# entn-at/exemplars_vc

Hardware: AMD Instinct MI355X
Metric: spectral frames/sec converted (100 NMF iters, N=4096 dict) (higher is better)
Workload: dtype f64

## Files before the change

exemplars_vc_amd/_lib.py:

```python
from __future__ import annotations

import ctypes as C
import os

_HERE = os.path.dirname(os.path.abspath(__file__))
LIB_PATH = os.environ.get("EVC_LIB") or os.path.join(_HERE, "libevc_hip.so")

F64, F32 = 0, 1
FRAME_MAJOR, BIN_MAJOR = 0, 1
EPS_ADD, EPS_ZERO_REPLACE, EPS_NONE, EPS_CLAMP = 0, 1, 2, 3
ALGO_GRAM, ALGO_FACTORED, ALGO_LITERAL, ALGO_AUTO = 0, 1, 2, 3
INIT_GIVEN, INIT_SKLEARN, INIT_CONST = 0, 1, 2
STOP_NONE, STOP_SKLEARN, STOP_PYMF, STOP_DECOMP = 0, 1, 2, 3
PROX_POSITIVE, PROX_SIGNED = 0, 1
PROX_ISTA, PROX_FISTA, PROX_NESTEROV = 0, 1, 2
PROX_LIP_MEAN, PROX_LIP_MAX = 0, 1
LOSS_FROBENIUS, LOSS_KL = 0, 1
FLAG_NO_FUSED, FLAG_EXACT_DIV, FLAG_NO_EXCHANGE, FLAG_NO_ALL_RESIDENT, FLAG_PAIR_TILES, FLAG_NO_LONE_BIN = 1, 2, 4, 16, 32, 64
LEARN_SKLEARN, LEARN_PYMF = 0, 1
CDL_BOTH, CDL_DICT_ONLY = 0, 1
DCL_BOTH, DCL_DICT_ONLY = 0, 1

SYMBOLS = ("evc_version", "evc_strerror", "evc_device_count", "evc_workspace_bytes",
           "evc_nmf_solve", "evc_nmf_convert", "evc_synthesize", "evc_residual",
           "evc_griffin_lim_workspace_bytes", "evc_griffin_lim", "evc_griffin_lim_batch_workspace_bytes",
           "evc_griffin_lim_batch", "evc_dtw_workspace_bytes", "evc_dtw_align",
           "evc_stft_frames", "evc_stft_workspace_bytes", "evc_stft", "evc_dict_bytes", "evc_dict_prepare",
           "evc_dtw_path_rows", "evc_dtw_gather_rows", "evc_cd_workspace_bytes", "evc_cd_solve",
           "evc_learn_workspace_bytes", "evc_learn_splits", "evc_nmf_learn",
           "evc_cd_learn_workspace_bytes", "evc_cd_learn_splits", "evc_cd_learn",
           "evc_mfcc_workspace_bytes", "evc_mfcc", "evc_beta_workspace_bytes", "evc_beta_solve",
           "evc_beta_learn_workspace_bytes", "evc_beta_learn_splits", "evc_beta_learn_route", "evc_beta_learn",
           "evc_online_workspace_bytes", "evc_online_splits", "evc_online_learn",
           "evc_online_transform_workspace_bytes", "evc_online_transform",
           "evc_online_fresh_workspace_bytes", "evc_online_learn_fresh",
           "evc_deconv_workspace_bytes", "evc_deconv_solve", "evc_deconv_synthesize",
           "evc_deconv_learn_workspace_bytes", "evc_deconv_learn_splits", "evc_deconv_learn",
           "evc_semi_workspace_bytes", "evc_semi_solve",
           "evc_prox_workspace_bytes", "evc_prox_solve",
           "evc_prox_masked_workspace_bytes", "evc_prox_masked_solve",
           "evc_prox_learn_workspace_bytes", "evc_prox_learn_block", "evc_prox_learn",
# ... 478 lines not shown
```

exemplars_vc_amd/csrc/evc_api.hip:

```cpp
#include "evc_solve_plan.h"

#include <math.h>
#include <stdlib.h>
#include <string.h>

using namespace evc;

namespace {

constexpr int DICT_MAGIC = 0x45564344;

struct SolveCall {
    const void* A; int lda;
    const void* X; int ldx;
    void* H; int ldh;
    int M, N, T_;
    const int* utt_offsets; int n_utt;
    void* ws; size_t ws_bytes;
    int* n_iter_out; double* err_out;
    const SynthArgs* y;
    hipStream_t s;
};

int copy_back(const UttState& u, int n_utt, int n_slots, int* n_iter_out, double* err_out, hipStream_t s) {
// ... 173 lines not shown
    inf->kernel = r.kernel;
    inf->members = r.members;
    inf->exchange = r.members > 1 ? 1 : 0;
    AbortHook hook(r.members > 1 ? fb.coop_cnt + COOP_MAX_TILES : nullptr, o.test_abort_at);
    HIP_TRY(hook.begin(true, s));
    int first = 1;
    if (o.check_every > 0 && o.stop_rule == EVC_STOP_SKLEARN) {
        HIP_TRY(fused_iterate(w.fl, fb, r, w.u, d.N, d.T_, 0, 1, 1, w.err2, o.eps_mode, o.eps, o.l1, 1, o.loss, s,
                              nullptr));
        HIP_TRY(utt_check(w.err2, w.u, n_utt, 0, o.check_every, o.stop_rule, o.tol, s));
        first = 0;
    }
    if (o.ev_loop_start) HIP_TRY(hipEventRecord((hipEvent_t)o.ev_loop_start, s));
    int done = 0;
    while (done < o.iters) {
        int n = o.iters - done;
        bool check = false;
        if (o.check_every > 0 && n >= o.check_every) { n = o.check_every; check = true; }
        const bool last = r.direct_export && done + n == o.iters;
        HIP_TRY(hook.before_launch(s));
        ++inf->launches;
        HIP_TRY(fused_iterate(w.fl, fb, r, w.u, d.N, d.T_, n, first, check ? 1 : 0, w.err2, o.eps_mode, o.eps, o.l1,
                              o.stop_rule == EVC_STOP_NONE ? 1 : 0, o.loss, s, last ? &lt : nullptr,
                              !(o.reserved & EVC_FLAG_NO_LONE_BIN)));
        first = 0;
        done += n;
        if (check)
            HIP_TRY(utt_check(w.err2, w.u, n_utt, done / o.check_every, o.check_every, o.stop_rule,
                              o.tol, s));
    }
    if (o.ev_loop_stop) HIP_TRY(hipEventRecord((hipEvent_t)o.ev_loop_stop, s));
    return ST_OK;
}

int finish_fused(const Workspace<double>& w, const Dims& d, const evc_solve_opts& o, const FusedTail& t, double* H, int ldh,
                 const SynthArgs* y, int y_members, hipStream_t s) {
    const bool fm = (o.layout == EVC_FRAME_MAJOR);
    if (t.export_h) HIP_TRY(fused_export_h(w.fl, w.fb.Hp, H, ldh, fm ? 1 : 0, d.T_, d.N, s));
    switch (t.y_from) {
        case Y_SLABS:
            return fused_unpack_y(w.flB, w.Yslab, y_members, (long)w.flB.vp, d.T_, y->Mb, static_cast<double*>(y->Y), y->ldy,
                                  fm ? 1 : 0, s);
        case Y_PREPASS:
            return fused_synthesize(w.flB, w.B2p, w.fb.Hp, w.Yp, w.u, d.N, d.T_, y->Mb, static_cast<double*>(y->Y), y->ldy,
                                    fm ? 1 : 0, s);
        case Y_ROWS:
            HIP_TRY(fused_export_h(w.fl, w.fb.Hp, w.H0, d.Np, 1, d.T_, d.N, s));
// ... 515 lines not shown
```

exemplars_vc_amd/csrc/evc_fused.hip:

```cpp
#include "evc_fused_common.h"

namespace evc {

__global__ void k_pack_dict(const double* __restrict__ At, int ldA, int n_rows, int NT, int msteps, int mtiles,
                            double* __restrict__ A1p, double* __restrict__ A2p, int ones_bin) {
    const long gid = (long)blockIdx.x * blockDim.x + threadIdx.x;
    const int msp = (msteps + 1) & ~1;
    const long n1 = (long)NT * msp * 64, n2 = (long)NT * mtiles * 4 * 64;
    if (gid < n1) {
        const int e = gid & 1, l = (gid >> 1) & 63, s = 2 * (int)((gid >> 7) % (msp / 2)) + e;
        const long j = (gid >> 7) / (msp / 2);
        const int i = l & 15;
        const long n = 16 * j + 4 * (i & 3) + (i >> 2);
        const int bin = bin_of(s, l >> 4);
        if (A1p) A1p[gid] = (s < msteps && bin == ones_bin) ? 1.0 : ((s < msteps && n < n_rows) ? At[n * ldA + bin] : 0.0);
    } else if (gid < n1 + n2) {
        const long g = gid - n1;
        const int e = g & 1, l = (g >> 1) & 63, r = 2 * (int)((g >> 7) & 1) + e, u = (g >> 8) % mtiles;
        const long j = (g >> 8) / mtiles;
        const long n = 16 * j + 4 * (l >> 4) + r;
        if (A2p) A2p[g] = n < n_rows ? At[n * ldA + 16 * u + (l & 15)] : 0.0;
    }
}

// ... 409 lines not shown

static hipError_t launch_general(const FusedLayout& f, const FusedArgs& a, int c_req, hipStream_t s) {
    const int C = a.skip_all_live ? 1 : (c_req > 0 ? c_req : (f.TT >= 1024 ? 2 : 1));
    switch (C) {
        case 1: return dispatch_msteps<1>(f.msteps, a, s);
        case 2: return dispatch_msteps<2>(f.msteps, a, s);
        default: return hipErrorInvalidValue;
    }
}

static FusedArgs fused_args(const FusedLayout& f, const double* A1p, const double* A2p, const double* Xp, const double* Hp,
                            double* Vp, const UttState& u, int N, int T_, int iters, int first) {
    FusedArgs a{};
    a.A1p = A1p; a.A2p = A2p; a.Xp = Xp; a.Hp = reinterpret_cast<f64x2*>(const_cast<double*>(Hp)); a.Vp = Vp;
    a.frame_utt = u.frame_utt; a.active = u.active;
    a.NT = f.NT; a.TT = f.TT; a.N = N; a.T_ = T_; a.M = f.M;
    a.iters = iters; a.first = first;
    a.coop_c = 1; a.spare_q = -1;
    return a;
}

hipError_t fused_iterate(const FusedLayout& f, const FusedBuffers& b, const FusedRoute& r, const UttState& u, int N,
                         int T_, int iters, int first, int write_err, double* err2, int eps_mode, double eps, double l1,
                         int all_live_known, int loss, hipStream_t s, const FusedLaunchTail* tail, bool lone_bin) {
    FusedArgs a = fused_args(f, b.A1p, b.A2p, b.Xp, b.Hp, b.Vp, u, N, T_, iters, first);
    a.err2 = err2; a.write_err = write_err;
    a.loss = loss; a.exact_div = r.exact_div;
    a.eps_mode = eps_mode; a.eps = eps; a.l1 = l1;
    const bool xy = r.kernel == EVC_KERNEL_FUSED_XY;
    const bool all_res = xy || r.kernel == EVC_KERNEL_FUSED_ALL;
    if (r.kernel == EVC_KERNEL_FUSED_MU) return launch_general(f, a, r.c_req, s);
    if (first && all_res && r.init_const && iters > 0) {
        a.init_const = 1; a.h0 = u.h0; a.rsum = b.rsum;
    } else if (first) {
        FusedArgs p = a;
        p.iters = 0;
        p.write_err = (iters == 0) ? write_err : 0;
        hipError_t e = launch_general(f, p, 1, s);
        if (e != hipSuccess) return e;
        a.first = 0;
    }
    if (iters == 0) return hipSuccess;
    hipError_t e;
    if (all_res) {
        a.coop_c = r.members; a.coop_buf = b.coop_buf; a.coop_cnt = b.coop_cnt;
        a.coop_abort = b.coop_cnt + COOP_MAX_TILES;
        if (all_live_known && tail) {
            a.Hx = tail->Hx; a.ldhx = tail->ldhx; a.hx_frame_major = tail->hx_frame_major;
            a.hx_wide = (a.Hx && a.hx_frame_major && !(reinterpret_cast<uintptr_t>(a.Hx) & 15) && !(a.ldhx & 1)) ? 1 : 0;
            if (!xy) {
                a.Yb2p = tail->Yb2p; a.Yslab = tail->Yslab; a.y_stride = tail->y_stride; a.y_mt = tail->y_mt;
                a.skip_hp = tail->skip_hp;
            }
        }
        e = xy ? fused_xy_launch(f.msteps, a, r.n_cus, s) : fused_all_launch(f.msteps, a, r.n_cus, s, lone_bin);
        a.coop_c = 1;
        a.first = 0; a.init_const = 0; a.Hx = nullptr; a.Yslab = nullptr; a.skip_hp = 0;
    } else {
        if (r.members > 1) {
            a.coop_c = r.members; a.coop_buf = b.coop_buf; a.coop_cnt = b.coop_cnt;
            a.coop_abort = b.coop_cnt + COOP_MAX_TILES;
        }
        e = fused_res_launch(f.msteps, a, s);
    }
    if (e != hipSuccess || all_live_known) return e;
    a.skip_all_live = 1;
    return launch_general(f, a, 1, s);
}

hipError_t fused_synthesize(const FusedLayout& fB, const double* B2p, const double* Hp, double* Yp,
                            const UttState& u, int N, int T_, int Mb, double* Y, long ldy, int frame_major,
                            hipStream_t s) {
    FusedArgs a = fused_args(fB, B2p, B2p, Yp, Hp, Yp, u, N, T_, 0, 1);
    a.force_live = 1; a.loss = EVC_LOSS_FROBENIUS; a.eps_mode = EVC_EPS_ADD;
    hipError_t e = dispatch_msteps<1>(fB.msteps, a, s);
    if (e != hipSuccess) return e;
    return fused_unpack_y(fB, Yp, 1, 0, T_, Mb, Y, ldy, frame_major, s);
}
// ... 11 lines not shown
```

exemplars_vc_amd/csrc/evc_fused_all_body.inc:

```
#if EVC_ALL_LONE
template <int MSTEPS, int C>
__global__ __launch_bounds__(ATHREADS, 2) void k_fused_lone(FusedArgs a) {
    constexpr bool KL = false, LONE = true;
    static_assert(MSTEPS > 4 && C > 1 && AllShape<MSTEPS, C, false>::LDS_DICT, "two bin tiles, the dictionary in LDS, direct exchange");
#else
template <int MSTEPS, int C, bool KL>
__global__ __launch_bounds__(ATHREADS, 2) void k_fused_all(FusedArgs a) {
    constexpr bool LONE = false;
#endif
    using S = AllShape<MSTEPS, C, KL>;
    constexpr int DS = LONE ? MSTEPS - 1 : MSTEPS;
    constexpr int MT = S::MT;
    constexpr int E = S::E;
    constexpr int NE = S::NE;
    constexpr int RSTR = S::RSTR;
    constexpr int MSP = (MSTEPS + 1) & ~1;
    constexpr int PR = S::PR;
    constexpr int TPD = 16 * PR;
    __shared__ __attribute__((aligned(16))) double s_red[2][AW * RSTR];
    __shared__ __attribute__((aligned(16))) double s_v[2][E];
    __shared__ __attribute__((aligned(16))) double s_x[2][E];
    __shared__ __attribute__((aligned(16))) double s_r[2][KL ? E : 1];
    __shared__ double s_stage[2][S::STG];
    __shared__ double s_dict[S::LDS_DICT ? ATILES * TPD : 1];
    __shared__ unsigned s_hb[2];
    __shared__ int s_fail;
    const int tid = threadIdx.x, lane = tid & 63;
    const int w8 = __builtin_amdgcn_readfirstlane(tid >> 6);
    const int half = w8 >> 2, w = w8 & 3, th = tid & (AW * 64 - 1);
    const int CR = C > 0 ? C : a.coop_c;
    const int member = blockIdx.x % CR;
    const int g = 2 * (blockIdx.x / CR) + half;
    double* const red = s_red[half];
    double* const vL = s_v[half];
    double* const xL = s_x[half];
    double* const rL = s_r[half];
    double* const stage = s_stage[half];
    unsigned hb = 0;
    const double* __restrict__ A1p = a.A1p;
    const double* __restrict__ A2p = a.A2p;
    f64x2* __restrict__ Hp = a.Hp;
    const int NT = a.NT;
    const long tile0 = (long)member * ATILES + w;
    const unsigned ul = (unsigned)lane;
    long sw = 0;

    const __amdgpu_buffer_rsrc_t r1 = __builtin_amdgcn_make_buffer_rsrc(const_cast<double*>(A1p), 0, NT * (MSP * 512), 0x00020000);
    const __amdgpu_buffer_rsrc_t r2 = __builtin_amdgcn_make_buffer_rsrc(const_cast<double*>(A2p), 0, NT * (MT * 2048), 0x00020000);
    const __amdgpu_buffer_rsrc_t rx = __builtin_amdgcn_make_buffer_rsrc(a.coop_buf, 0, C > 1 ? 2 * a.groups * (C * 4096) : 0, 0x00020000);
// ... 54 lines not shown
                }
            return;
        }
#ifdef EVC_ALL_NOFRAG
        if (nofrag_go) return;
#endif
        const int so = (int)(tile0 + sw + AW * k) * (MT * 2048);
#pragma unroll
        for (int u = 0; u < MT; ++u)
#pragma unroll
            for (int r = 0; r < 4; r += 2) {
                const f64x2 v = __builtin_bit_cast(f64x2, __builtin_amdgcn_raw_buffer_load_b128(r2, ul16 + (u * 2 + (r >> 1)) * 1024, so, 0));
                a2[u][r] = v[0];
                a2[u][r + 1] = v[1];
            }
    };

    const int mode = a.eps_mode;
    const double eps = a.eps;
    const double d0 = a.l1 + (mode == EVC_EPS_ADD ? a.eps : 0.0);
    const f64x4 dinit = {d0, d0, d0, d0};
    const unsigned lo = fast_lo(mode, eps);
    unsigned seq = 0;
    int rs_es = 1, rs_len = 0, rs_pub0 = 0, rs_pub1 = 0, rs_src0 = -1, rs_src1 = -1, rs_src2 = -1;
    if (C < 0) {
        rs_es = (NE + CR - 1) / CR;
        rs_len = NE - member * rs_es;
        rs_len = rs_len < 0 ? 0 : (rs_len > rs_es ? rs_es : rs_len);
        const int e0 = th, e1 = th + AW * 64;
        const int j0 = e0 / rs_es, j1 = (e1 < NE ? e1 : e0) / rs_es;
        rs_pub0 = (j0 * CR + member) * rs_es + (e0 - j0 * rs_es);
        rs_pub1 = (j1 * CR + member) * rs_es + ((e1 < NE ? e1 : e0) - j1 * rs_es);
        auto src = [&](int idx) {
            if (idx >= CR * rs_es) return -1;
            const int el = idx % rs_es;
            return el < rs_len ? member * CR * rs_es + idx : -1;
        };
        rs_src0 = src(th);
        rs_src1 = src(th + AW * 64);
        rs_src2 = src(th + 2 * AW * 64);
    }
    if (tid == 0) s_fail = 0;
    if (tid < 2) s_hb[tid] = 0;

    if (a.stagger_cycles > 0 && ((blockIdx.x / CR) & 1)) {
        const long long t0 = __builtin_amdgcn_s_memtime();
// ... 31 lines not shown
            }
            const double hv = h0_of(lane & 15);
#pragma unroll
            for (int k = 0; k < AKT; ++k) {
                const long n0 = 16 * (tile0 + AW * k) + 4 * (lane >> 4);
#pragma unroll
                for (int r = 0; r < 4; ++r) h[k][r] = n0 + r < a.N ? hv : 0.0;
            }
        } else if (valid) {
            for (int e = th; e < E; e += AW * 64) {
                const int s = e >> 6, l = e & 63;
                const bool in = s < MSTEPS;
                xL[e] = in ? a.Xp[(tt * MSTEPS + s) * 64 + l] : 0.0;
                vL[e] = in ? a.Vp[(tt * 8 + s) * 64 + l] : 0.0;
                if (KL) rL[e] = xL[e] / (vL[e] < a.eps ? a.eps : vL[e]);
            }
#pragma unroll
            for (int k = 0; k < AKT; ++k) {
                const f64x2* t = Hp + (tt * NT + tile0 + AW * k) * 128;
                const f64x2 h01 = t[ul], h23 = t[ul + 64];
                h[k][0] = h01[0]; h[k][1] = h01[1]; h[k][2] = h23[0]; h[k][3] = h23[1];
            }
        }
        __syncthreads();
        if (valid && !KL) {
            double x[DS], xl = 0.0;
#pragma unroll
            for (int s = 0; s < DS; ++s) x[s] = xL[s * 64 + lane];
            if constexpr (LONE) xl = xL[DS * 64 + (lane & 15)];
            load_a1(a1, 0, lds);
            if constexpr (LONE) load_lone(al, 0);
#pragma unroll
            for (int k = 0; k < AKT; ++k) {
                f64x4 acc = {0, 0, 0, 0};
                if constexpr (LONE) {
#pragma unroll
                    for (int r = 0; r < 4; ++r) acc[r] = al[r] * xl;
                }
#pragma unroll
                for (int s = 0; s < DS; ++s) acc = Mma<double>::mma(a1[s], x[s], acc);
                if (!decltype(lds)::value || k + 1 < AKT) load_a1(a1, (k + 1) % AKT, lds);
                if constexpr (LONE) {
                    if (k + 1 < AKT) load_lone(al, k + 1);
                }
                p[k] = acc;
            }
        }

        if (valid && KL) load_a1(a1, 0, lds);
        for (int step = 0; step <= 2 * a.iters; ++step) {
#ifdef EVC_ALL_NOFRAG
            nofrag_go = step > 2;
#endif
            const bool mine = C == 1 ? (step & 1) == 0 : (step & 1) == half;
            EVC_STAMP(0);
            if (valid && mine && step < 2 * a.iters) {
                asm volatile("" : "+s"(sw));
                double v[DS], vl = 0.0;
#pragma unroll
                for (int s = 0; s < DS; ++s) v[s] = KL ? rL[s * 64 + lane] : vL[s * 64 + lane];
                if constexpr (LONE) vl = vL[DS * 64 + (lane & 15)];
                if constexpr (decltype(lds)::value) load_a1(a1, 0, lds);
                f64x4 dl = dinit;
                if constexpr (LONE) {
                    load_lone(al, 0);
#pragma unroll
                    for (int r = 0; r < 4; ++r) dl[r] = __builtin_fma(al[r], vl, d0);
                }
                f64x4 vn[MT];
#pragma unroll
                for (int u = 0; u < MT; ++u) vn[u] = f64x4{0, 0, 0, 0};
#pragma unroll
                for (int k = 0; k < AKT; ++k) {
                    __builtin_amdgcn_sched_barrier(0);
                    load_a2(a2, k, lds);
                    f64x4 d = KL ? f64x4{0, 0, 0, 0} : (LONE ? dl : dinit);
#pragma unroll
                    for (int s = 0; s < DS; ++s) d = Mma<double>::mma(a1[s], v[s], d);
                    if (!decltype(lds)::value || k + 1 < AKT)
                        load_a1(a1, (k + 1) % AKT, lds);
                    if constexpr (LONE) {
                        if (k + 1 < AKT) load_lone(al, k + 1);
                    }
                    __builtin_amdgcn_sched_barrier(0);
                    if constexpr (LONE) {
                        if (k + 1 < AKT) {
#pragma unroll
                            for (int r = 0; r < 4; ++r) dl[r] = __builtin_fma(al[r], vl, d0);
                        }
                    }
                    if (KL) {
#pragma unroll
                        for (int r = 0; r < 4; ++r) h[k][r] *= d[r];
                    } else {
                        mu_tile_guarded(h[k], p[k], d, mode, eps, lo);
                    }
#pragma unroll
                    for (int u = 0; u < MT; ++u)
#pragma unroll
                        for (int r = 0; r < 4; ++r) vn[u] = Mma<double>::mma(a2[u][r], h[k][r], vn[u]);
                }
#pragma unroll
                for (int u = 0; u < MT; ++u)
#pragma unroll
                    for (int r = 0; r < 4; ++r)
                        if (u * 4 + r < MSTEPS) red[w * RSTR + (u * 4 + r) * 64 + lane] = vn[u][r];
            } else if (C > 1 && valid && !mine && step > 0) {
                __builtin_amdgcn_s_setprio(ALL_EXCH_PRIO);
                const bool act = th < NE / 2;
                const int ep = act ? 2 * th : 0;
                f64x2 sm = {0.0, 0.0};
                if (w * 64 < NE / 2) {
                    f64x2 pv[AW];
#pragma unroll
                    for (int ww = 0; ww < AW; ++ww) pv[ww] = *reinterpret_cast<const f64x2*>(red + ww * RSTR + ep);
                    static_assert(AW == 4, "the four partials are named one by one");
                    asm volatile("" : "+v"(pv[0]), "+v"(pv[1]), "+v"(pv[2]), "+v"(pv[3]));
#pragma unroll
                    for (int ww = 0; ww < AW; ++ww) sm += pv[ww];
                    const long long tag = (seq >> 1) & 1;
                    const long long m0 = (__double_as_longlong(sm[0]) & ~1LL) | tag;
                    const long long m1 = (__double_as_longlong(sm[1]) & ~1LL) | tag;
                    const int xo = __builtin_amdgcn_readfirstlane((int)(((seq & 1) * (unsigned)a.groups + (unsigned)g) * (unsigned)(C * 4096)));
                    if (act)
                        __builtin_amdgcn_raw_buffer_store_b128(__builtin_bit_cast(all_u32x4, all_i64x2{m0, m1}), rx, ep * 8,
                                                               xo + member * 4096, 16);
                    bool ok = true;
                    unsigned polls = 0;
                    {
                        const long long* sp = reinterpret_cast<const long long*>(a.coop_buf) +
                                              ((size_t)(seq & 1) * a.groups + g) * (size_t)(C * 512) +
                                              (lane < C ? lane : 0) * 512 + (NE - 1);
                        for (;;) {
                            const long long b = __hip_atomic_load(sp, __ATOMIC_RELAXED, __HIP_MEMORY_SCOPE_AGENT);
// ... 14 lines not shown
                        for (int m = 0; m < C; ++m)
                            if (m != member)
                                b[m] = __builtin_bit_cast(all_i64x2, __builtin_amdgcn_raw_buffer_load_b128(rx, ep * 8, xo + m * 4096, 16));
                        long long bad = 0;
#pragma unroll
                        for (int m = 0; m < C; ++m) {
                            b[m] = (m == member) ? all_i64x2{m0, m1} : b[m];
                            bad |= (b[m][0] ^ tag) | (b[m][1] ^ tag);
                        }
                        if ((bad & 1) == 0) break;
                        if (all_polls_out(polls, a.coop_abort)) {
                            ok = false;
                            break;
                        }
                        __builtin_amdgcn_s_sleep(2);
                    }
                    f64x2 v2 = {0.0, 0.0};
#pragma unroll
                    for (int m = 0; m < C; ++m) {
                        v2[0] += __longlong_as_double(b[m][0] & ~1LL);
                        v2[1] += __longlong_as_double(b[m][1] & ~1LL);
                    }
                    if (!ok) s_fail = 1;
                    if (act) {
                        *reinterpret_cast<f64x2*>(vL + ep) = v2;
                        if (KL) {
                            const f64x2 x2 = *reinterpret_cast<const f64x2*>(xL + ep);
                            *reinterpret_cast<f64x2*>(rL + ep) =
                                f64x2{x2[0] / (v2[0] < a.eps ? a.eps : v2[0]), x2[1] / (v2[1] < a.eps ? a.eps : v2[1])};
                        }
                    }
                }
                ++seq;
                __builtin_amdgcn_s_setprio(0);
            } else if (valid && !mine && step > 0) {
                const int e0 = C <= 0 ? th % NE : th, e1 = th + AW * 64;
                const bool has1 = e1 < NE;
                __builtin_amdgcn_s_setprio(ALL_EXCH_PRIO);
                double s0 = 0.0, s1 = 0.0;
#pragma unroll
                for (int ww = 0; ww < AW; ++ww) {
                    s0 += red[ww * RSTR + e0];
                    s1 += red[ww * RSTR + (has1 ? e1 : e0)];
                }
                if (C < 0) {
                    long long* xb1 = reinterpret_cast<long long*>(a.coop_buf) +
                                     ((size_t)(seq & 1) * a.groups + g) * (size_t)CR * ALL_RS_STRIDE;
                    long long* xb2 = reinterpret_cast<long long*>(a.coop_buf) + ALL_SLICE_OFFSET +
                                     ((size_t)(seq & 1) * a.groups + g) * 512;
                    const long long tag = (seq >> 1) & 1;
                    __hip_atomic_store(xb1 + rs_pub0, (__double_as_longlong(s0) & ~1LL) | tag, __ATOMIC_RELAXED,
                                       __HIP_MEMORY_SCOPE_AGENT);
                    if (has1)
                        __hip_atomic_store(xb1 + rs_pub1, (__double_as_longlong(s1) & ~1LL) | tag, __ATOMIC_RELAXED,
// ... 82 lines not shown
                            __hip_atomic_fetch_add(&s_hb[half], 1u, __ATOMIC_RELEASE, __HIP_MEMORY_SCOPE_WORKGROUP);
                        while ((int)(__hip_atomic_load(&s_hb[half], __ATOMIC_ACQUIRE, __HIP_MEMORY_SCOPE_WORKGROUP) - hb) < 0)
                            __builtin_amdgcn_s_sleep(1);
                        if (th < 4 * ES) {
                            const int el = th >> 2, q = th & 3, per = CR >> 2;
                            double v = 0.0;
                            for (int i = 0; i < per; ++i) v += stage[(q * per + i) * ES + el];
                            v += __shfl_xor(v, 1, 64);
                            v += __shfl_xor(v, 2, 64);
                            if (q == 0)
                                __hip_atomic_store(xb2 + member * ES + el, (__double_as_longlong(v) & ~1LL) | tag,
                                                   __ATOMIC_RELAXED, __HIP_MEMORY_SCOPE_AGENT);
                        }
                    }
                    long long g0, g1;
                    fetch2(xb2 + e0, xb2 + (has1 ? e1 : e0), g0, g1);
                    s0 = __longlong_as_double(g0 & ~1LL);
                    s1 = __longlong_as_double(g1 & ~1LL);
                    ++seq;
                    if (!ok) s_fail = 1;
                }
                vL[e0] = s0;
                if (has1) vL[e1] = s1;
                if (KL) {
                    rL[e0] = xL[e0] / (s0 < a.eps ? a.eps : s0);
                    if (has1) rL[e1] = xL[e1] / (s1 < a.eps ? a.eps : s1);
                }
                __builtin_amdgcn_s_setprio(0);
            }
            EVC_STAMP(1);
            __syncthreads();
            EVC_STAMP(2);
            if (C != 1 && s_fail) {
                if (tid == 0) __hip_atomic_store(a.coop_abort, 1, __ATOMIC_RELAXED, __HIP_MEMORY_SCOPE_AGENT);
                return;
            }
        }

        auto y_tail = [&](auto ut) __attribute__((always_inline)) {
            constexpr int UT = decltype(ut)::value;
            f64x4 yn[UT];
#pragma unroll
            for (int u = 0; u < UT; ++u) yn[u] = f64x4{0, 0, 0, 0};
            if (valid) {
                const __amdgpu_buffer_rsrc_t rb = __builtin_amdgcn_make_buffer_rsrc(const_cast<double*>(a.Yb2p), 0, NT * (UT * 2048), 0x00020000);
#pragma unroll
// ... 69 lines not shown
                    }
                }
            }
            if (member == 0) {
                for (int e = th; e < NE; e += AW * 64) a.Vp[(tt * 8 + (e >> 6)) * 64 + (e & 63)] = vL[e];
                if (a.write_err && w == 0) {
                    double e = 0.0;
#pragma unroll
                    for (int s = 0; s < MSTEPS; ++s) {
                        const double x = xL[s * 64 + lane], vv = vL[s * 64 + lane];
                        e += KL ? kl_terms(x, vv, a.eps) : (x - vv) * (x - vv);
                    }
                    e += __shfl_xor(e, 16, 64);
                    e += __shfl_xor(e, 32, 64);
                    const long t = 16 * tt + lane;
                    if (lane < 16 && t < a.T_) a.err2[t] = e;
                }
            }
        }
        __syncthreads();
    }
    };

    if constexpr (S::LDS_DICT) {
        if (LONE ? a.M == 4 * MSTEPS - 3 : (a.M > 0 && a.M < PR)) {
            for (int x = tid; x < ATILES * TPD; x += ATHREADS) {
                const int slot = x / TPD, e = all_dict_row((x / PR) % 16), b = x % PR;
                const long j = (long)member * ATILES + slot / AKT + AW * (slot % AKT);
                const int q = e >> 2, r = e & 3;
                s_dict[x] = b < a.M ? A2p[((j * MT + (b >> 4)) * 2 + (r >> 1)) * 128 + (16 * q + (b & 15)) * 2 + (r & 1)] : 0.0;
            }
            __syncthreads();
            run(std::true_type{});
            return;
        }
    }
    if constexpr (!LONE) run(std::false_type{});
}
```

exemplars_vc_amd/csrc/evc_fused_common.h:

```cpp
#pragma once
#include "evc_internal.h"

#include <type_traits>

namespace evc {

typedef double f64x2 __attribute__((ext_vector_type(2)));

__host__ __device__ inline int fused_msteps(int M) { return M <= 16 ? (M + 3) / 4 : 4 + (M - 16 + 3) / 4; }
__device__ __forceinline__ int bin_of(int s, int q) { return 16 * (s >> 2) + q + 4 * (s & 3); }

struct FusedArgs {
    const double* A1p;
    const double* A2p;
    const double* Xp;
    f64x2* Hp;
    double* Vp;
    double* err2;
    const int* frame_utt;
    const int* active;
    int NT, TT, N, T_;
    int iters;
    int first;
    int write_err;
    int skip_all_live;
    int force_live;
    int exact_div;
    int loss;
    int eps_mode;
    double eps, l1;
    int coop_c;
    double* coop_buf;
    int* coop_cnt;
    int* coop_abort;
    int groups;
    int init_const;
    const double* h0;
    const double* rsum;
    double* Hx;
    long ldhx;
    int hx_frame_major;
    int hx_wide;
    const double* Yb2p;
    double* Yslab;
    long y_stride;
    int y_mt;
    int skip_hp;
    int M, spare_q;
    long long stagger_cycles;
#if defined(EVC_ALL_TIMING) || defined(EVC_XY_TIMING)
    long long* dbg;
#endif
};

// ... 63 lines not shown
template <class HT>
__device__ __forceinline__ void mu_tile_guarded(HT& h, const f64x4& p, const f64x4& dacc, int mode, double eps, unsigned lo) {
    const unsigned span = FAST_HI_WORD > lo ? FAST_HI_WORD - lo : 0u;
    const unsigned worst = max(max(hi_word(dacc[0]) - lo, hi_word(dacc[1]) - lo),
                               max(hi_word(dacc[2]) - lo, hi_word(dacc[3]) - lo));
    double rc[4], q[4];
    batch_rcp(dacc, rc);
#pragma unroll
    for (int r = 0; r < 4; ++r) q[r] = p[r] * rc[r];
    if (__builtin_expect(!__all(worst < span), 0)) {
#pragma unroll
        for (int r = 0; r < 4; ++r) {
            double dn = dacc[r];
            dn = (mode == EVC_EPS_ZERO_REPLACE && dn == 0.0) ? eps : dn;
            dn = (mode == EVC_EPS_CLAMP && !(dn > eps)) ? eps : dn;
            q[r] = p[r] / dn;
            __builtin_amdgcn_sched_barrier(0);
        }
    }
#pragma unroll
    for (int r = 0; r < 4; ++r) h[r] = h[r] * q[r];
}

hipError_t fused_res_launch(int msteps, const FusedArgs& a, hipStream_t s);
hipError_t fused_all_launch(int msteps, const FusedArgs& a, int n_cus, hipStream_t s, bool lone_bin = true);
hipError_t fused_xy_launch(int msteps, const FusedArgs& a, int n_cus, hipStream_t s);

__device__ __forceinline__ double kl_terms(double x, double v, double eps) {
    double e = v;
    if (x > eps) e += x * log(x / (v < eps ? eps : v)) - x;
    return 2.0 * e;
}

}
```

exemplars_vc_amd/csrc/evc_internal.h:

```cpp
#pragma once
#include <hip/hip_runtime.h>
#include <stdint.h>
#include "../../include/evc.h"

namespace evc {

typedef double f64x4 __attribute__((ext_vector_type(4)));
typedef float f32x4 __attribute__((ext_vector_type(4)));

template <typename T> struct Mma;
template <> struct Mma<double> {
    typedef f64x4 acc_t;
    static __device__ __forceinline__ acc_t mma(double a, double b, acc_t c) {
        return __builtin_amdgcn_mfma_f64_16x16x4f64(a, b, c, 0, 0, 0);
    }
    static __device__ __forceinline__ int row(int lane, int r) { return (lane >> 4) + 4 * r; }
};
template <> struct Mma<float> {
    typedef f32x4 acc_t;
    static __device__ __forceinline__ acc_t mma(float a, float b, acc_t c) {
        return __builtin_amdgcn_mfma_f32_16x16x4f32(a, b, c, 0, 0, 0);
    }
    static __device__ __forceinline__ int row(int lane, int r) { return 4 * (lane >> 4) + r; }
};
// ... 233 lines not shown
    double* Yslab;
    long y_stride;
    int y_mt;
    int skip_hp;
};
bool fused_supported(int M, int N, int T_, int dtype);
FusedLayout fused_layout(int M, int N, int T_);
hipError_t fused_pack_dict(const FusedLayout& f, double* A1p, double* A2p, const double* At, int ldA, int n_rows,
                           hipStream_t s, int ones_bin = -1);
hipError_t fused_pack_frames(const FusedLayout& f, double* Xp, const double* Xt, int ldx, hipStream_t s);
hipError_t fused_rowsum(const double* At, int ldA, int M, int N, double* rsum, hipStream_t s);
hipError_t fused_import_h(const FusedLayout& f, double* Hp, const double* H, long ldh, int frame_major, int T_,
                          int N, hipStream_t s);
hipError_t fused_export_h(const FusedLayout& f, const double* Hp, double* H, long ldh, int frame_major, int T_,
                          int N, hipStream_t s);
hipError_t fused_fill_h(const FusedLayout& f, double* Hp, int N, int T_, const UttState& u, hipStream_t s);
hipError_t fused_synthesize(const FusedLayout& fB, const double* B2p, const double* Hp, double* Yp,
                            const UttState& u, int N, int T_, int Mb, double* Y, long ldy, int frame_major,
                            hipStream_t s);
hipError_t fused_unpack_y(const FusedLayout& fB, const double* Yp, int members, long stride, int T_, int Mb, double* Y,
                          long ldy, int frame_major, hipStream_t s);
hipError_t fused_iterate(const FusedLayout& f, const FusedBuffers& b, const FusedRoute& r, const UttState& u, int N,
                         int T_, int iters, int first, int write_err, double* err2, int eps_mode, double eps, double l1,
                         int all_live_known, int loss, hipStream_t s, const FusedLaunchTail* tail, bool lone_bin = true);

struct WideLayout {
    int MT;
    int W;
    int NB;
    int TT, G;
    int c, rmode;
    int tagged;
    size_t aw, xw, hw, vpart, vsum;
};
struct WideBuffers {
    float *Aw, *Xw, *Hw, *Pw, *Vpart, *Vsum;
    unsigned* ctl;
    float* Hs;
    size_t hs_stride;
    double* err2s;
    long err_stride;
    int snap_slots;
};
bool wide_supported(int M, int N, int T_, int dtype, int algo);
WideLayout wide_layout(int M, int N, int T_, int n_cus, int c_req, int w_req);
size_t wide_ctl_words(const WideLayout& f);
struct WideCaps { size_t aw, xw, hw, vpart, vsum, ctl; int c_cap; };
// ... 135 lines not shown
```

exemplars_vc_amd/solver.py:

```python
from __future__ import annotations

import contextlib
import ctypes as C
import os
import threading
import types
from typing import Optional, Sequence

import numpy as np

from . import _lib

_EPS_MODES = {"add": _lib.EPS_ADD, "zero_replace": _lib.EPS_ZERO_REPLACE, "none": _lib.EPS_NONE,
              "clamp": _lib.EPS_CLAMP}
_EPS_DEFAULT = {"add": 1e-9, "zero_replace": float(np.finfo(np.float32).eps), "none": 0.0,
                "clamp": 1e-15}
_ALGOS = {"gram": _lib.ALGO_GRAM, "factored": _lib.ALGO_FACTORED, "literal": _lib.ALGO_LITERAL,
          "auto": _lib.ALGO_AUTO}
_INITS = {"given": _lib.INIT_GIVEN, "sklearn": _lib.INIT_SKLEARN, "const": _lib.INIT_CONST}
_STOPS = {"none": _lib.STOP_NONE, "sklearn": _lib.STOP_SKLEARN, "pymf": _lib.STOP_PYMF}
_PROX_STOPS = {"none": _lib.STOP_NONE, "decomp": _lib.STOP_DECOMP}
_PROX_MOMENTA = {"ista": _lib.PROX_ISTA, "fista": _lib.PROX_FISTA, "nesterov": _lib.PROX_NESTEROV}
_LAYOUTS = {"frame_major": _lib.FRAME_MAJOR, "bin_major": _lib.BIN_MAJOR}
_LOSSES = {"frobenius": _lib.LOSS_FROBENIUS, "kullback-leibler": _lib.LOSS_KL, "kl": _lib.LOSS_KL}
# ... 258 lines not shown
    if not info:
        return None, None, None, None
    n_iter, trace = np.zeros(n_utt, dtype=np.int32), np.full((n_utt, width), np.nan)
    return n_iter, trace, n_iter.ctypes.data_as(C.POINTER(C.c_int)), trace.ctypes.data_as(C.POINTER(C.c_double))


def _call(L, entry, device, head, ws_bytes=None, tail=()):
    torch = _torch()
    lease = _workspace(ws_bytes, device) if ws_bytes is not None else contextlib.nullcontext()
    with torch.cuda.device(device), lease as ws:
        stream = C.c_void_p(torch.cuda.current_stream(device).cuda_stream)
        if ws is None:
            st = getattr(L, entry)(*head, *tail, stream)
        else:
            st = getattr(L, entry)(*head, ws.data_ptr(), ws.numel(), *tail, stream)
    _lib.check(st, entry)


def _solve(A, X, H0, B, *, layout="bin_major", iters=100, eps_mode="add", eps=None,
           l1=0.0, algo="auto", init=None, init_value=0.0, check_every=0,
           stop_rule="none", tol=0.0, utt_offsets: Optional[Sequence[int]] = None,
           dtype=None, device=None, info=False, out=None, loop_events=None,
           fused=True, fused_c=0, fused_w=0, want_h=True, out_y=None, loss="frobenius", exact_div=False,
           cooperative=True, all_resident=True, pair_tiles=False, lone_bin=True, _fake_coop_timeout=False, solve_info=None):
    torch = _torch()
    device = require_device(device)
    L = _lib.lib()
    lay = _LAYOUTS[layout]
    pd = A if isinstance(A, PreparedDictionary) else None
    if pd is not None:
        if dtype is None:
            dtype = pd.tdtype
        if pd.device != device:
            raise ValueError("the prepared dictionary lives on another device")
        if _pick_dtype(dtype)[1] != pd.dcode or _LOSSES[loss] != pd.loss:
            raise ValueError("the prepared dictionary was made for another dtype / loss")
    p = _operands(A, X, H0, init, layout, dtype, device, utt_offsets, out, want_h or B is None)
    tdtype, dcode, A_d, X_d, H_d, M, N, T, n_utt = p.tdtype, p.dcode, p.A_d, p.X_d, p.H_d, p.M, p.N, p.T, p.n_utt
    Mb = 0
    B_d = None
    if B is True:
        if pd is None or pd.Mb == 0:
            raise ValueError("convert() without B needs a prepared dictionary that holds B")
        Mb = pd.Mb
    elif B is not None:
        B_d, _ = _to_dev(B, tdtype, device)
        Mb, N2 = B_d.shape if lay == _lib.BIN_MAJOR else B_d.shape[::-1]
        if N2 != N:
            raise ValueError(f"A and B disagree on the number of exemplars: {N} vs {N2}")
    if B is not None:
        yshape = (Mb, T) if lay == _lib.BIN_MAJOR else (T, Mb)
        Y_d = out_y if out_y is not None else torch.empty(yshape, dtype=tdtype, device=device)

    opts = _lib.SolveOpts()
    opts.algo = _ALGOS[algo]
    opts.iters, opts.eps_mode, opts.init_mode = int(iters), _EPS_MODES[eps_mode], _INITS[p.init]
    opts.check_every, opts.stop_rule = int(check_every), _STOPS[stop_rule]
    opts.eps = _EPS_DEFAULT[eps_mode] if eps is None else float(eps)
    opts.l1, opts.tol, opts.init_value = float(l1), float(tol), float(init_value)
    opts.loss = _LOSSES[loss]
    opts.reserved = ((0 if fused else _lib.FLAG_NO_FUSED) | (_lib.FLAG_EXACT_DIV if exact_div else 0)
                     | (0 if cooperative else _lib.FLAG_NO_EXCHANGE)
                     | (0 if all_resident else _lib.FLAG_NO_ALL_RESIDENT) | (_lib.FLAG_PAIR_TILES if pair_tiles else 0)
                     | (0 if lone_bin else _lib.FLAG_NO_LONE_BIN)
                     | ((int(fused_c) & 0xff) << 8)
                     | ((int(fused_w) & 0xf) << 16))
    if _fake_coop_timeout is not False and _fake_coop_timeout is not None:
        opts.test_abort_at = -1 if _fake_coop_timeout is True else int(_fake_coop_timeout)
    sinfo = _lib.SolveInfo()
    sinfo.struct_bytes = C.sizeof(_lib.SolveInfo)
    opts.info = C.addressof(sinfo)
    if pd is not None:
        if loss in ("kl", "kullback-leibler") and opts.eps != pd.eps:
            raise ValueError("the prepared dictionary's KL guard differs from this call's eps")
        opts.dict = C.addressof(pd.handle)
    _common_opts(opts, dcode, lay, loop_events)

    ws_bytes = int(L.evc_workspace_bytes(M, Mb, N, T, n_utt, dcode, opts.algo))
    n_iter, err, ni_p, er_p = _trace_arrays(n_utt, _n_slots(iters, check_every), info)
    h_args = (H_d.data_ptr(), _ld(H_d)) if H_d is not None else (None, 0)
    ax_args = ((A_d.data_ptr(), _ld(A_d)) if A_d is not None else (None, 0)) + (X_d.data_ptr(), _ld(X_d))
    if B is None:
        entry, head = "evc_nmf_solve", (*ax_args, *h_args, M, N, T)
    else:
        b_args = (B_d.data_ptr(), _ld(B_d)) if B_d is not None else (None, 0)
        entry, head = "evc_nmf_convert", (*ax_args, *b_args, *h_args, Y_d.data_ptr(), _ld(Y_d), M, Mb, N, T)
    _call(L, entry, device, (*head, p.off_ptr, n_utt, C.byref(opts)), ws_bytes, (ni_p, er_p))
# ... 1222 lines not shown
```

include/evc.h:

```cpp
#ifndef EVC_H
#define EVC_H

#include <stddef.h>

#ifdef __cplusplus
extern "C" {
#endif

#define EVC_VERSION 100

typedef struct ihipStream_t* evc_stream_t;

enum { EVC_F64 = 0, EVC_F32 = 1 };

enum { EVC_FRAME_MAJOR = 0, EVC_BIN_MAJOR = 1 };

enum { EVC_EPS_ADD = 0, EVC_EPS_ZERO_REPLACE = 1, EVC_EPS_NONE = 2, EVC_EPS_CLAMP = 3 };

enum { EVC_ALGO_GRAM = 0, EVC_ALGO_FACTORED = 1, EVC_ALGO_LITERAL = 2, EVC_ALGO_AUTO = 3 };

enum { EVC_INIT_GIVEN = 0, EVC_INIT_SKLEARN = 1, EVC_INIT_CONST = 2 };

enum { EVC_STOP_NONE = 0, EVC_STOP_SKLEARN = 1, EVC_STOP_PYMF = 2, EVC_STOP_DECOMP = 3 };

enum { EVC_LOSS_FROBENIUS = 0, EVC_LOSS_KL = 1 };

enum { EVC_FLAG_NO_FUSED = 1, EVC_FLAG_EXACT_DIV = 2, EVC_FLAG_NO_EXCHANGE = 4, EVC_FLAG_NO_ALL_RESIDENT = 16, EVC_FLAG_PAIR_TILES = 32,
       EVC_FLAG_NO_LONE_BIN = 64 };

struct evc_solve_info;
struct evc_dict;
typedef struct evc_solve_opts {
    int struct_bytes;
    int dtype;
    int layout;
    int algo;
    int iters;
    int eps_mode;
    int init_mode;
    int check_every;
    int stop_rule;
    int reserved;
    int loss;
    int test_abort_at;
    double eps;
    double l1;
    double tol;
    double init_value;
    void* ev_loop_start;
    void* ev_loop_stop;
    struct evc_solve_info* info;
// ... 458 lines not shown
```

Before: 1.005 million.

## Hoist denominator range guard in fused MU update via dictionary and V range proofs

Adds a one-time per-block check that dictionary columns are nonnegative with bounded sums, plus a per-iteration wave vote that the reconstruction V values fall inside a safe exponent range, both published through shared memory. When both hold, the multiplicative update skips the per-tile exact-division guard and relies only on the fast reciprocal. This is meant to remove guard compare-and-branch work from the inner update loop, at the cost of an extra shared-memory flag exchange, a column-sum pass at kernel start, and more complexity. It is on by default and can be disabled with a new flag.

```diff
diff --git a/exemplars_vc_amd/_lib.py b/exemplars_vc_amd/_lib.py
--- a/exemplars_vc_amd/_lib.py
+++ b/exemplars_vc_amd/_lib.py
@@ -17,6 +17,7 @@
 PROX_LIP_MEAN, PROX_LIP_MAX = 0, 1
 LOSS_FROBENIUS, LOSS_KL = 0, 1
 FLAG_NO_FUSED, FLAG_EXACT_DIV, FLAG_NO_EXCHANGE, FLAG_NO_ALL_RESIDENT, FLAG_PAIR_TILES, FLAG_NO_LONE_BIN = 1, 2, 4, 16, 32, 64
+FLAG_NO_RANGE_HOIST = 128
 LEARN_SKLEARN, LEARN_PYMF = 0, 1
 CDL_BOTH, CDL_DICT_ONLY = 0, 1
 DCL_BOTH, DCL_DICT_ONLY = 0, 1
diff --git a/exemplars_vc_amd/csrc/evc_api.hip b/exemplars_vc_amd/csrc/evc_api.hip
--- a/exemplars_vc_amd/csrc/evc_api.hip
+++ b/exemplars_vc_amd/csrc/evc_api.hip
@@ -219,7 +219,7 @@
         ++inf->launches;
         HIP_TRY(fused_iterate(w.fl, fb, r, w.u, d.N, d.T_, n, first, check ? 1 : 0, w.err2, o.eps_mode, o.eps, o.l1,
                               o.stop_rule == EVC_STOP_NONE ? 1 : 0, o.loss, s, last ? &lt : nullptr,
-                              !(o.reserved & EVC_FLAG_NO_LONE_BIN)));
+                              !(o.reserved & EVC_FLAG_NO_LONE_BIN), !(o.reserved & EVC_FLAG_NO_RANGE_HOIST)));
         first = 0;
         done += n;
         if (check)
diff --git a/exemplars_vc_amd/csrc/evc_fused.hip b/exemplars_vc_amd/csrc/evc_fused.hip
--- a/exemplars_vc_amd/csrc/evc_fused.hip
+++ b/exemplars_vc_amd/csrc/evc_fused.hip
@@ -455,7 +455,8 @@
 
 hipError_t fused_iterate(const FusedLayout& f, const FusedBuffers& b, const FusedRoute& r, const UttState& u, int N,
                          int T_, int iters, int first, int write_err, double* err2, int eps_mode, double eps, double l1,
-                         int all_live_known, int loss, hipStream_t s, const FusedLaunchTail* tail, bool lone_bin) {
+                         int all_live_known, int loss, hipStream_t s, const FusedLaunchTail* tail, bool lone_bin,
+                         bool range_hoist) {
     FusedArgs a = fused_args(f, b.A1p, b.A2p, b.Xp, b.Hp, b.Vp, u, N, T_, iters, first);
     a.err2 = err2; a.write_err = write_err;
     a.loss = loss; a.exact_div = r.exact_div;
@@ -486,7 +487,9 @@
                 a.skip_hp = tail->skip_hp;
             }
         }
+        a.range_hoist = (!xy && range_hoist) ? 1 : 0;
         e = xy ? fused_xy_launch(f.msteps, a, r.n_cus, s) : fused_all_launch(f.msteps, a, r.n_cus, s, lone_bin);
+        a.range_hoist = 0;
         a.coop_c = 1;
         a.first = 0; a.init_const = 0; a.Hx = nullptr; a.Yslab = nullptr; a.skip_hp = 0;
     } else {
diff --git a/exemplars_vc_amd/csrc/evc_fused_all_body.inc b/exemplars_vc_amd/csrc/evc_fused_all_body.inc
--- a/exemplars_vc_amd/csrc/evc_fused_all_body.inc
+++ b/exemplars_vc_amd/csrc/evc_fused_all_body.inc
@@ -10,6 +10,7 @@
 #endif
     using S = AllShape<MSTEPS, C, KL>;
     constexpr int DS = LONE ? MSTEPS - 1 : MSTEPS;
+    constexpr bool HOIST = !KL && C >= 1;
     constexpr int MT = S::MT;
     constexpr int E = S::E;
     constexpr int NE = S::NE;
@@ -25,6 +26,7 @@
     __shared__ double s_dict[S::LDS_DICT ? ATILES * TPD : 1];
     __shared__ unsigned s_hb[2];
     __shared__ int s_fail;
+    __shared__ __attribute__((aligned(16))) unsigned s_vok[HOIST ? 2 : 1][HOIST ? AW : 1];
     const int tid = threadIdx.x, lane = tid & 63;
     const int w8 = __builtin_amdgcn_readfirstlane(tid >> 6);
     const int half = w8 >> 2, w = w8 & 3, th = tid & (AW * 64 - 1);
@@ -125,6 +127,7 @@
     const f64x4 dinit = {d0, d0, d0, d0};
     const unsigned lo = fast_lo(mode, eps);
     unsigned seq = 0;
+    bool tame = false;
     int rs_es = 1, rs_len = 0, rs_pub0 = 0, rs_pub1 = 0, rs_src0 = -1, rs_src1 = -1, rs_src2 = -1;
     if (C < 0) {
         rs_es = (NE + CR - 1) / CR;
@@ -202,6 +205,9 @@
                 h[k][0] = h01[0]; h[k][1] = h01[1]; h[k][2] = h23[0]; h[k][3] = h23[1];
             }
         }
+        if constexpr (HOIST) {
+            if (lane == 0) s_vok[half][w] = 0u;
+        }
         __syncthreads();
         if (valid && !KL) {
             double x[DS], xl = 0.0;
@@ -238,8 +244,17 @@
                 asm volatile("" : "+s"(sw));
                 double v[DS], vl = 0.0;
 #pragma unroll
-                for (int s = 0; s < DS; ++s) v[s] = KL ? rL[s * 64 + lane] : vL[s * 64 + lane];
+                for (int s = 0; s < DS; ++s) {
+                    v[s] = KL ? rL[s * 64 + lane] : vL[s * 64 + lane];
+                    if constexpr (HOIST && MSTEPS == 2 && decltype(lds)::value) LDS_NO_PAIR();
+                }
                 if constexpr (LONE) vl = vL[DS * 64 + (lane & 15)];
+                bool safe = false;
+                if constexpr (HOIST) {
+                    static_assert(AW == 4, "the half's four words are one 16-byte read");
+                    const all_u32x4 ok4 = *reinterpret_cast<const all_u32x4*>(s_vok[half]);
+                    safe = tame && __builtin_amdgcn_readfirstlane((int)(ok4[0] & ok4[1] & ok4[2] & ok4[3])) != 0;
+                }
                 if constexpr (decltype(lds)::value) load_a1(a1, 0, lds);
                 f64x4 dl = dinit;
                 if constexpr (LONE) {
@@ -272,6 +287,8 @@
                     if (KL) {
 #pragma unroll
                         for (int r = 0; r < 4; ++r) h[k][r] *= d[r];
+                    } else if constexpr (HOIST) {
+                        mu_tile_hoisted(h[k], p[k], d, mode, eps, lo, safe);
                     } else {
                         mu_tile_guarded(h[k], p[k], d, mode, eps, lo);
                     }
@@ -290,6 +307,7 @@
                 const bool act = th < NE / 2;
                 const int ep = act ? 2 * th : 0;
                 f64x2 sm = {0.0, 0.0};
+                unsigned vok = 1u;
                 if (w * 64 < NE / 2) {
                     f64x2 pv[AW];
 #pragma unroll
@@ -350,6 +368,10 @@
                         v2[1] += __longlong_as_double(b[m][1] & ~1LL);
                     }
                     if (!ok) s_fail = 1;
+                    if constexpr (HOIST) {
+                        const bool real = act && bin_of(ep >> 6, (ep & 63) >> 4) < a.M;
+                        vok = __all(!real || (range_v_ok(v2[0]) && range_v_ok(v2[1]))) ? 1u : 0u;
+                    }
                     if (act) {
                         *reinterpret_cast<f64x2*>(vL + ep) = v2;
                         if (KL) {
@@ -358,6 +380,9 @@
                                 f64x2{x2[0] / (v2[0] < a.eps ? a.eps : v2[0]), x2[1] / (v2[1] < a.eps ? a.eps : v2[1])};
                         }
                     }
+                }
+                if constexpr (HOIST) {
+                    if (lane == 0) s_vok[half][w] = vok;
                 }
                 ++seq;
                 __builtin_amdgcn_s_setprio(0);
@@ -486,6 +511,12 @@
                 }
                 vL[e0] = s0;
                 if (has1) vL[e1] = s1;
+                if constexpr (HOIST) {
+                    const bool real0 = e0 < NE && bin_of(e0 >> 6, (e0 & 63) >> 4) < a.M;
+                    const bool real1 = has1 && bin_of(e1 >> 6, (e1 & 63) >> 4) < a.M;
+                    const unsigned vok = __all((!real0 || range_v_ok(s0)) && (!real1 || range_v_ok(s1))) ? 1u : 0u;
+                    if (lane == 0) s_vok[half][w] = vok;
+                }
                 if (KL) {
                     rL[e0] = xL[e0] / (s0 < a.eps ? a.eps : s0);
                     if (has1) rL[e1] = xL[e1] / (s1 < a.eps ? a.eps : s1);
@@ -601,6 +632,23 @@
     }
     };
 
+    if constexpr (HOIST) {
+        static_assert(ATHREADS == 16 * ATILES, "one thread per exemplar of the member");
+        const long j = (long)member * ATILES + (tid >> 4);
+        const int e = tid & 15, q = e >> 2, r = e & 3;
+        bool ok = a.range_hoist != 0 && a.M > 0 && a.M <= 16 * MT && 16 * j + e < a.N && d0 >= 0.0 && d0 <= RANGE_SUM_HI &&
+                  lo <= RANGE_LO_MAX;
+        if (ok) {
+            double cs = 0.0;
+            for (int b = 0; b < a.M; ++b) {
+                const double x = A2p[((j * MT + (b >> 4)) * 2 + (r >> 1)) * 128 + (16 * q + (b & 15)) * 2 + (r & 1)];
+                ok = ok && x >= 0.0;
+                cs += x;
+            }
+            ok = ok && cs >= RANGE_SUM_LO && cs <= RANGE_SUM_HI;
+        }
+        tame = __builtin_amdgcn_readfirstlane(__syncthreads_and(ok)) != 0;
+    }
     if constexpr (S::LDS_DICT) {
         if (LONE ? a.M == 4 * MSTEPS - 3 : (a.M > 0 && a.M < PR)) {
             for (int x = tid; x < ATILES * TPD; x += ATHREADS) {
diff --git a/exemplars_vc_amd/csrc/evc_fused_common.h b/exemplars_vc_amd/csrc/evc_fused_common.h
--- a/exemplars_vc_amd/csrc/evc_fused_common.h
+++ b/exemplars_vc_amd/csrc/evc_fused_common.h
@@ -30,6 +30,7 @@
     int eps_mode;
     double eps, l1;
     int coop_c;
+    int range_hoist;
     double* coop_buf;
     int* coop_cnt;
     int* coop_abort;
@@ -139,6 +140,37 @@
     for (int r = 0; r < 4; ++r) h[r] = h[r] * q[r];
 }
 
+constexpr unsigned RANGE_V_LO = 0x39B00000u;
+constexpr unsigned RANGE_V_HI = 0x46300000u;
+constexpr unsigned RANGE_LO_MAX = 0x33600000u;
+constexpr double RANGE_SUM_LO = 0x1p-100, RANGE_SUM_HI = 0x1p100;
+__device__ __forceinline__ bool range_v_ok(double x) { return hi_word(x) - RANGE_V_LO < RANGE_V_HI - RANGE_V_LO; }
+template <class HT>
+__device__ __forceinline__ void mu_tile_hoisted(HT& h, const f64x4& p, const f64x4& dacc, int mode, double eps, unsigned lo,
+                                                bool safe) {
+    double rc[4], q[4];
+    batch_rcp(dacc, rc);
+#pragma unroll
+    for (int r = 0; r < 4; ++r) q[r] = p[r] * rc[r];
+    if (__builtin_expect(!safe, 0)) {
+        const unsigned span = FAST_HI_WORD > lo ? FAST_HI_WORD - lo : 0u;
+        const unsigned worst = max(max(hi_word(dacc[0]) - lo, hi_word(dacc[1]) - lo),
+                                   max(hi_word(dacc[2]) - lo, hi_word(dacc[3]) - lo));
+        if (__builtin_expect(!__all(worst < span), 0)) {
+#pragma unroll
+            for (int r = 0; r < 4; ++r) {
+                double dn = dacc[r];
+                dn = (mode == EVC_EPS_ZERO_REPLACE && dn == 0.0) ? eps : dn;
+                dn = (mode == EVC_EPS_CLAMP && !(dn > eps)) ? eps : dn;
+                q[r] = p[r] / dn;
+                __builtin_amdgcn_sched_barrier(0);
+            }
+        }
+    }
+#pragma unroll
+    for (int r = 0; r < 4; ++r) h[r] = h[r] * q[r];
+}
+
 hipError_t fused_res_launch(int msteps, const FusedArgs& a, hipStream_t s);
 hipError_t fused_all_launch(int msteps, const FusedArgs& a, int n_cus, hipStream_t s, bool lone_bin = true);
 hipError_t fused_xy_launch(int msteps, const FusedArgs& a, int n_cus, hipStream_t s);
diff --git a/exemplars_vc_amd/csrc/evc_internal.h b/exemplars_vc_amd/csrc/evc_internal.h
--- a/exemplars_vc_amd/csrc/evc_internal.h
+++ b/exemplars_vc_amd/csrc/evc_internal.h
@@ -279,7 +279,8 @@
                           long ldy, int frame_major, hipStream_t s);
 hipError_t fused_iterate(const FusedLayout& f, const FusedBuffers& b, const FusedRoute& r, const UttState& u, int N,
                          int T_, int iters, int first, int write_err, double* err2, int eps_mode, double eps, double l1,
-                         int all_live_known, int loss, hipStream_t s, const FusedLaunchTail* tail, bool lone_bin = true);
+                         int all_live_known, int loss, hipStream_t s, const FusedLaunchTail* tail, bool lone_bin = true,
+                         bool range_hoist = true);
 
 struct WideLayout {
     int MT;
diff --git a/exemplars_vc_amd/solver.py b/exemplars_vc_amd/solver.py
--- a/exemplars_vc_amd/solver.py
+++ b/exemplars_vc_amd/solver.py
@@ -304,7 +304,8 @@
            stop_rule="none", tol=0.0, utt_offsets: Optional[Sequence[int]] = None,
            dtype=None, device=None, info=False, out=None, loop_events=None,
            fused=True, fused_c=0, fused_w=0, want_h=True, out_y=None, loss="frobenius", exact_div=False,
-           cooperative=True, all_resident=True, pair_tiles=False, lone_bin=True, _fake_coop_timeout=False, solve_info=None):
+           cooperative=True, all_resident=True, pair_tiles=False, lone_bin=True, range_hoist=True, _fake_coop_timeout=False,
+           solve_info=None):
     torch = _torch()
     device = require_device(device)
     L = _lib.lib()
@@ -344,7 +345,7 @@
     opts.reserved = ((0 if fused else _lib.FLAG_NO_FUSED) | (_lib.FLAG_EXACT_DIV if exact_div else 0)
                      | (0 if cooperative else _lib.FLAG_NO_EXCHANGE)
                      | (0 if all_resident else _lib.FLAG_NO_ALL_RESIDENT) | (_lib.FLAG_PAIR_TILES if pair_tiles else 0)
-                     | (0 if lone_bin else _lib.FLAG_NO_LONE_BIN)
+                     | (0 if lone_bin else _lib.FLAG_NO_LONE_BIN) | (0 if range_hoist else _lib.FLAG_NO_RANGE_HOIST)
                      | ((int(fused_c) & 0xff) << 8)
                      | ((int(fused_w) & 0xf) << 16))
     if _fake_coop_timeout is not False and _fake_coop_timeout is not None:
diff --git a/include/evc.h b/include/evc.h
--- a/include/evc.h
+++ b/include/evc.h
@@ -26,7 +26,7 @@
 enum { EVC_LOSS_FROBENIUS = 0, EVC_LOSS_KL = 1 };
 
 enum { EVC_FLAG_NO_FUSED = 1, EVC_FLAG_EXACT_DIV = 2, EVC_FLAG_NO_EXCHANGE = 4, EVC_FLAG_NO_ALL_RESIDENT = 16, EVC_FLAG_PAIR_TILES = 32,
-       EVC_FLAG_NO_LONE_BIN = 64 };
+       EVC_FLAG_NO_LONE_BIN = 64, EVC_FLAG_NO_RANGE_HOIST = 128 };
 
 struct evc_solve_info;
 struct evc_dict;
```

Measured after the change: 1.034 million (median of 6 runs). 1.03x the previous value.
